# ga1i13o/DiffewS

Hardware: AMD Instinct MI355X
Metric: few-shot episodes/sec (512x512, 1-shot, SD-2 UNet) (higher is better)
Workload: dtype bf16; 1 GPU; SD-2.1 UNet + SD VAE, 512x512, 1-shot, 4 episodes/GPU/step (BASELINE.json configs[1]); nshot=1, resolution=512, parallelism=episode-sharded x1, hip_graph=True, residual_dtype=bf16, graph_owner=pipeline.run_episodes(captured=True)

## Files before the change

### diffews_amd/_lib.py

```python
import ctypes as C
import os

_HERE = os.path.dirname(os.path.abspath(__file__))
LIB_PATH = os.environ.get("DFW_LIB") or os.path.join(_HERE, "libdiffews_hip.so")

BF16, F16 = 0, 1
FILTER_BILINEAR, FILTER_BICUBIC = 0, 1
OUT_T, OUT_F32, OUT_NCHW_F32 = 0, 1, 2
ACT_NONE, ACT_SILU, ACT_CLAMP1 = 0, 1, 2

_vp, _i32, _i64, _f32, _sz = C.c_void_p, C.c_int32, C.c_int64, C.c_float, C.c_size_t


class GemmArgs(C.Structure):
    _fields_ = [("A", _vp), ("W", _vp), ("C", _vp), ("bias", _vp), ("rowbias", _vp), ("residual", _vp),
                ("workspace", _vp), ("workspace_bytes", _sz), ("a_elems", _i64), ("w_elems", _i64),
                ("M", _i32), ("N", _i32), ("K", _i32), ("lda", _i32), ("ldc", _i32), ("ldr", _i32), ("ld_rowbias", _i32),
                ("taps", _i32), ("Cin", _i32), ("Hi", _i32), ("Wi", _i32), ("Ho", _i32), ("Wo", _i32),
                ("stride", _i32), ("pad", _i32), ("ups", _i32), ("rows_per_img", _i32),
                ("out_scale", _f32), ("act", _i32), ("geglu", _i32), ("out_mode", _i32), ("splitk", _i32),
                ("batch", _i32), ("strideA", _i64), ("strideW", _i64), ("strideC", _i64), ("dtype", _i32),
                ("gn_partial", _vp), ("gn_groups", _i32),
                ("colscale", _f32), ("colscale_n", _i32), ("residual_f32", _i32), ("W_blocked", _vp)]

# ... 159 lines not shown
    _fields_ = [("q", _vp), ("k", _vp), ("v", _vp), ("out", _vp),
                ("batch", _i32), ("n", _i32), ("head_dim", _i32), ("q_prescaled", _i32),
                ("ldq", _i32), ("ldk", _i32), ("ldv", _i32), ("ldo", _i32),
                ("q_bs", _i64), ("k_bs", _i64), ("v_bs", _i64), ("o_bs", _i64), ("dtype", _i32)]


class AdamWArgs(C.Structure):
    _fields_ = [("param", _vp), ("grad", _vp), ("exp_avg", _vp), ("exp_avg_sq", _vp), ("grad_sumsq", _vp), ("n", _i64),
                ("lr", _f32), ("beta1", _f32), ("beta2", _f32), ("eps", _f32), ("weight_decay", _f32), ("max_grad_norm", _f32),
                ("step", _i32), ("shadow", _vp), ("shadow_dtype", _i32), ("found_inf", _vp)]


class Config(C.Structure):
    _fields_ = [("conv_patch", _i32), ("big_kernels", _i32), ("big_bm", _i32), ("big_bn", _i32), ("big_bk", _i32),
                ("gemm_bm", _i32), ("gemm_bn", _i32), ("fsa_key_split", _i32),
                ("fsa_force_splits", _i32), ("big_min_tiles", _i32), ("k8", _i32)]


SYMBOLS = {
    "dfw_configure": (_i32, [C.POINTER(Config)]),
    "dfw_get_config": (None, [C.POINTER(Config)]),
    "dfw_version": (_i32, []),
    "dfw_error_string": (C.c_char_p, [_i32]),
    "dfw_graph_memset_nodes": (_i32, [_vp, C.POINTER(_i32)]),
    "dfw_gemm": (_i32, [C.POINTER(GemmArgs), _vp]),
    "dfw_gemm_workspace_bytes": (_sz, [C.POINTER(GemmArgs)]),
    "dfw_gemm_kernel_name": (_i32, [C.POINTER(GemmArgs), C.c_char_p, _sz]),
    "dfw_gemm_gn_chunks": (_i32, [C.POINTER(GemmArgs)]),
    "dfw_conv_up2x": (_i32, [C.POINTER(ConvUp2xArgs), _vp]),
    "dfw_conv_up2x_kernel_name": (_i32, [C.POINTER(ConvUp2xArgs), C.c_char_p, _sz]),
    "dfw_conv_up2x_gn_chunks": (_i32, [C.POINTER(ConvUp2xArgs)]),
    "dfw_fsa_attention": (_i32, [C.POINTER(FsaArgs), _vp]),
    "dfw_fsa_workspace_bytes": (_sz, [C.POINTER(FsaArgs)]),
    "dfw_fsa_kernel_name": (_i32, [C.POINTER(FsaArgs), C.c_char_p, _sz]),
    "dfw_fsa_attention_sets": (_i32, [C.POINTER(FsaArgs), _i32, _vp]),
    "dfw_fsa_sets_kernel_name": (_i32, [C.POINTER(FsaArgs), _i32, C.c_char_p, _sz]),
    "dfw_fsa_attention_ragged": (_i32, [C.POINTER(FsaArgs), C.POINTER(_i32), _i32, _i32, _vp]),
    "dfw_fsa_ragged_kernel_name": (_i32, [C.POINTER(FsaArgs), C.POINTER(_i32), _i32, _i32, C.c_char_p, _sz]),
    "dfw_fsa_ragged_workspace_bytes": (_sz, [C.POINTER(FsaArgs), C.POINTER(_i32), _i32, _i32]),
    "dfw_fsa_attention_routed": (_i32, [C.POINTER(FsaArgs), _vp, C.POINTER(_i32), _i32, _i32, _vp]),
    "dfw_fsa_routed_kernel_name": (_i32, [C.POINTER(FsaArgs), _i32, _i32, C.c_char_p, _sz]),
    "dfw_fsa_routed_workspace_bytes": (_sz, [C.POINTER(FsaArgs), _i32, _i32]),
    "dfw_cross_attention": (_i32, [C.POINTER(XattnArgs), _vp]),
# ... 109 lines not shown
```

### diffews_amd/csrc/gemm.hip

```cpp
#include "gemm_common.h"
#include <stdio.h>
#include <stdlib.h>

namespace dfw {

template <typename T, int BM, int BN, bool CONV, bool RF32 = false>
__global__ __launch_bounds__(256, 2) void gemm_kernel(const GemmP p) {
  constexpr int WTM = BM / 2, WTN = BN / 2, MB = WTM / 32, NB = WTN / 32;
  constexpr int SA = BM / 32, SW = BN / 32;
  constexpr int BUF = (BM + BN) * 128;
  extern __shared__ __attribute__((aligned(16))) char smem[];

  const int tid = threadIdx.x, lane = tid & 63, wave = tid >> 6;
  const int wm = wave >> 1, wn = wave & 1;
  const int lr = lane & 31, lh = lane >> 5;

  const int ntiles = p.ntm * p.ntn;
  const int nxb = gridDim.x >> 3, xcd = blockIdx.x & 7;
  const int Q = (ntiles + 7) >> 3;
  const int t_end = min(ntiles, (xcd + 1) * Q);
  int tile = xcd * Q + (blockIdx.x >> 3);

  const int z = blockIdx.y;
  int ks0 = 0, ks1 = p.nk;
// ... 270 lines not shown
  const int zdim = p.batch > 1 ? p.batch : (p.splitk > 1 ? p.splitk : 1);
  int nwg = q.ntm * q.ntn;
  int cap = 256 * per_cu / (zdim < 4 ? zdim : 4);
  if (cap < 256) cap = 256;
  if (nwg > cap) nwg = cap;
  nwg = (nwg + 7) & ~7;
  dim3 grid(nwg, zdim);
  if (p.taps == 1) {
    if (pl.rf32) hipLaunchKernelGGL((gemm_kernel<T, BM, BN, false, true>), grid, dim3(256), lds, st, q);
    else hipLaunchKernelGGL((gemm_kernel<T, BM, BN, false>), grid, dim3(256), lds, st, q);
  } else {
    if (pl.rf32) hipLaunchKernelGGL((gemm_kernel<T, BM, BN, true, true>), grid, dim3(256), lds, st, q);
    else hipLaunchKernelGGL((gemm_kernel<T, BM, BN, true>), grid, dim3(256), lds, st, q);
  }
  DFW_CHECK_LAUNCH();
  if (p.splitk > 1) {
    const long long total = (long long)p.M * (p.N >> 2);
    int blocks = (int)((total + 255) / 256);
    if (blocks > 2048) blocks = 2048;
    hipLaunchKernelGGL((splitk_reduce_kernel<T>), dim3(blocks), dim3(256), 0, st, q);
    DFW_CHECK_LAUNCH();
  }
  return 0;
}

struct TileCost { int bm, bn; float R, L, E; };
static const TileCost kTiles[3] = {{128, 128, 1.67f, 0.70f, 0.f}, {128, 64, 2.8f, 0.50f, 0.f}, {64, 64, 3.7f, 0.40f, 0.f}};
static const TileCost kLinTiles[3] = {{128, 128, 5.29f, 0.312f, 1.94f}, {128, 64, 8.52f, 0.182f, 0.13f}, {64, 64, 12.9f, 0.145f, 0.f}};

static void plan_gemm(GemmP& p, int& bm, int& bn) {
  const int fbm = cfg().gemm_bm, fbn = cfg().gemm_bn;
  const bool fixed_sk = p.splitk >= 1;
  if (p.geglu) { bm = 128; bn = 128; p.splitk = 1; return; }
  const bool can_split = p.batch <= 1 && (p.N % 4) == 0;
  float best = 1e30f;
  int best_t = 0, best_sk = 1;
  for (int t = 0; t < 3; ++t) {
// ... 127 lines not shown
  p.splitk = splitk; p.batch = batch;
  p.res_f32 = a->residual_f32 ? 1 : 0;
  p.strideA = a->strideA; p.strideW = a->strideW; p.strideC = a->strideC;
  p.nk = a->K / 64; p.cpt = a->Cin / 64; p.ntn = 0; p.ntm = 0;
  p.dtype_bf16 = a->dtype == DFW_BF16;
  p.gn_partial = a->gn_partial; p.gn_groups = a->gn_groups; p.gn_chunks = 0;
#ifdef DFW_TILE_STAMPS
  p.stamps = nullptr; p.stamp_tiles = 0;
#endif
  p.conv_chunk_major = a->taps == 9 ? 1 : 0;
  if (p.splitk > p.nk) p.splitk = p.nk;
  plan_gemm(p, p.plan_bm, p.plan_bn);
  return 0;
}

static int plan_call(const dfw_gemm_args* a, GemmP& p, GemmPlan& pl) {
  const int rc = fill_params(a, p);
  if (rc == 0) pl = gemm_plan(p);
  return rc;
}

extern "C" int dfw_gemm_kernel_name(const dfw_gemm_args* a, char* buf, size_t n) {
  GemmP p;
  GemmPlan pl;
  const int rc = plan_call(a, p, pl);
  if (rc) return rc;
  if (!buf || n == 0) return DFW_EINVAL;
  const char *t = p.dtype_bf16 ? "bf16" : "f16", *k = p.taps == 9 ? "conv" : "lin";
  switch (pl.kernel) {
    case GemmKernel::K8: snprintf(buf, n, "gemm8_kernel<%s,256,%d,64,%s>", t, pl.bn, k); break;
// ... 37 lines not shown
```

### diffews_amd/csrc/gemm8.hip

```cpp
#include "gemm_common.h"
#include <type_traits>

namespace dfw {

template <typename T, bool CONV, int BN, bool UP2X = false>
__global__ __launch_bounds__(512, 2) void gemm8_kernel(const GemmP p) {
  constexpr int BM = 256, HT = 16384;
  static_assert(!UP2X || (CONV && BN != 160), "the folded upsample conv is a conv mode of the 256 / 128 wide tiles");
  constexpr int KW = UP2X ? 4 : 1;
  constexpr bool N160 = BN == 160;
  static_assert(!(N160 && CONV), "the 256 x 160 tile is instantiated for Linear shapes only");
  constexpr int WH = BN / 128;
  constexpr int WGN = N160 ? 2 : BN / 64, WGM = 8 / WGN;
  constexpr int NBW = N160 ? 5 : 4;
  constexpr int WTM = BM / WGM, MB6 = WTM / 16, MH = MB6 / 2;
  constexpr int WDMA = N160 ? 3 : 2 * WH;
  constexpr int WB160 = 65536, WS160 = 24576;
  constexpr int STG = N160 ? WB160 + 2 * WS160 : (2 + WH) * 32768;
  extern __shared__ __attribute__((aligned(16))) char smem[];
  const int tid = threadIdx.x, lane = tid & 63;
  const int wave = __builtin_amdgcn_readfirstlane(tid >> 6);
  const int wr = wave >> 2;
  const int wm = wave / WGN, wc = wave % WGN;
  const uint32_t lds0 = lds_addr(smem);

  const int ntiles = p.ntm * p.ntn;
  const int nxb = gridDim.x >> 3, xcd = blockIdx.x & 7;
  const int Q = (ntiles + 7) >> 3;
  const int t_end = min(ntiles, (xcd + 1) * Q);
  const int tile0 = xcd * Q + (blockIdx.x >> 3);
  if (tile0 >= t_end) return;
  const int my_tiles = (t_end - tile0 + nxb - 1) / nxb;
  const int nkt = p.K >> 6;
  const int cpt = p.Cin >> 6;

  const int z = blockIdx.y;
  const char* Ab = p.A;
  const char* Wb = p.W;
  char* Cb = p.C;
  if (p.batch > 1) {
    Ab += (size_t)z * p.strideA * sizeof(T);
    Wb += (size_t)z * p.strideW * sizeof(T);
    Cb += (size_t)z * p.strideC * sizeof(T);
  }
  const u32x4 ra = make_srd(Ab, p.a_bytes);
  const u32x4 rw = make_srd(Wb, p.w_bytes);

  auto tile_coords = [&](int t) -> TileC {
    TileC c;
    c.par = 0;
    if constexpr (UP2X) {
      c.par = t & 3;
      t >>= 2;
    }
    const int tn = t % p.ntn, tm = t / p.ntn;
    c.m0 = tm * BM;
    c.n0 = tn * BN;
    c.img = 0; c.oy0 = 0; c.ox0 = 0;
    if constexpr (CONV) {
      c.img = tm / p.tpi;
      const int t2 = tm - c.img * p.tpi, tyi = t2 / p.tpr, txi = t2 - tyi * p.tpr;
      c.oy0 = tyi << 4;
      c.ox0 = txi << 4;
    }
    return c;
  };
  auto row_to_m = [&](const TileC& c, int r) -> int {
    if constexpr (UP2X) return (c.img * p.Ho + 2 * (c.oy0 + (r >> 4)) + (c.par >> 1)) * p.Wo + 2 * (c.ox0 + (r & 15)) + (c.par & 1);
    else if constexpr (CONV) return (c.img * p.Ho + c.oy0 + (r >> 4)) * p.Wo + c.ox0 + (r & 15);
    else return c.m0 + r;
  };

  const int lrow = lane >> 3;
  const int kc = (lane & 7) ^ ((((wave & 1) << 2) + (lane >> 4)) & 7);
  const unsigned limH = p.ups ? 2 * p.Hi : p.Hi, limW = p.ups ? 2 * p.Wi : p.Wi;
  const int ush = p.ups ? 1 : 0;
  int a_kt = 0, a_ti = 0;
  bool a_live = true;
  uint32_t a_v0 = 0;
  int a_m = 0, a_ix0 = 0;
  int a_iy0 = 0;
  uint32_t a_pix = 0;
  auto a_setup = [&](const TileC& c) {
    if constexpr (!CONV) {
      a_m = c.m0 + wave * 8 + lrow;
      a_v0 = (uint32_t)(((size_t)a_m * p.lda + kc * 8) * sizeof(T));
    } else {
      a_iy0 = (c.oy0 + (wave >> 1)) * p.stride - p.pad;
      a_ix0 = (c.ox0 + (wave & 1) * 8 + lrow) * p.stride - p.pad;
      a_pix = (uint32_t)c.img * (uint32_t)(p.Hi * p.Wi);
      if constexpr (UP2X) {
        a_iy0 += c.par >> 1;
        a_ix0 += c.par & 1;
      }
    }
  };
  auto a_advance = [&]() {
    if (++a_kt == nkt) {
      a_kt = 0;
      if (++a_ti < my_tiles) a_setup(tile_coords(tile0 + a_ti * nxb));
      else a_live = false;
    }
  };
  auto issue_a = [&](int buf) __attribute__((always_inline)) {
    int ky = 0, kx = 0, cc = 0;
    if constexpr (UP2X) {
      cc = a_kt >> 2;
      ky = (a_kt >> 1) & 1;
      kx = a_kt & 1;
    } else if constexpr (CONV) {
      cc = a_kt / 9;
      const int tap = a_kt - cc * 9;
      ky = tap / 3;
      kx = tap - ky * 3;
    }
#pragma unroll
    for (int h = 0; h < 2; ++h) {
      const uint32_t dst = lds0 + (uint32_t)(h * 32768 + buf * HT) + (uint32_t)wave * 1024u;
#pragma unroll
      for (int j = 0; j < 2; ++j) {
        uint32_t off;
        if constexpr (!CONV) {
          const int dr = h * 128 + j * 64;
          off = (a_m + dr < p.M && a_live) ? a_v0 + (uint32_t)dr * (uint32_t)p.lda * (uint32_t)sizeof(T) + (uint32_t)a_kt * 128u : kOOB;
        } else {
          int iy = a_iy0 + (h * 8 + j * 4) * p.stride + ky, ix = a_ix0 + kx;
          const bool ok = (unsigned)iy < limH && (unsigned)ix < limW && a_live;
          iy >>= ush;
          ix >>= ush;
          off = ok ? ((a_pix + (uint32_t)(iy * p.Wi + ix)) * (uint32_t)p.lda + (uint32_t)(cc * 64 + kc * 8)) * (uint32_t)sizeof(T) : kOOB;
        }
        dma16(ra, off, dst + j * 8192);
      }
    }
    a_advance();
  };
  int w_kt = 0, w_ti = 0;
  bool w_live = true;
  uint32_t w_v0 = 0;
  int w_n = 0, w_par = 0;
  auto w_setup = [&](const TileC& c) {
    w_n = c.n0 + wave * 8 + lrow;
    w_par = c.par;
    w_v0 = (uint32_t)(((size_t)w_n * p.K * KW + kc * 8) * sizeof(T));
  };
  auto issue_w = [&](int buf) __attribute__((always_inline)) {
    uint32_t koff = (uint32_t)w_kt * 128u;
    if constexpr (UP2X) {
      const int cc = w_kt >> 2, tap = w_kt & 3;
      koff = (uint32_t)((w_par * 4 + tap) * p.Cin + cc * 64) * (uint32_t)sizeof(T);
    } else if constexpr (CONV) {
      const int cc = w_kt / 9, tap = w_kt - cc * 9;
      koff = (uint32_t)(tap * p.Cin + cc * 64) * (uint32_t)sizeof(T);
    }
    if constexpr (N160) {
      const uint32_t dst = lds0 + (uint32_t)(WB160 + buf * WS160) + (uint32_t)wave * 1024u;
#pragma unroll
      for (int j = 0; j < 3; ++j) {
// ... 1 lines not shown
        const bool ok = w_live && (j < 2 || wave < 4);
        dma16(rw, ok ? off : kOOB, dst + j * 8192);
      }
    }
#pragma unroll
    for (int h = 0; h < (N160 ? 0 : WH); ++h) {
      const uint32_t dst = lds0 + (uint32_t)((2 + h) * 32768 + buf * HT) + (uint32_t)wave * 1024u;
#pragma unroll
      for (int j = 0; j < 2; ++j) {
        const uint32_t off = w_v0 + (uint32_t)(h * 128 + j * 64) * (uint32_t)(p.K * KW) * (uint32_t)sizeof(T) + koff;
        bool ok = w_live;
        if constexpr (BN == 128) ok = ok && (w_n + j * 64 < p.N);
        dma16(rw, ok ? off : kOOB, dst + j * 8192);
      }
    }
    if (++w_kt == nkt) {
      w_kt = 0;
      if (++w_ti < my_tiles) {
        if (UP2X || p.ntn > 1) w_setup(tile_coords(tile0 + w_ti * nxb));
      } else w_live = false;
    }
  };

  uint32_t ab0, ab1, wb0, wb1;
  {
    const int l15 = lane & 15, l4 = lane >> 4;
    const uint32_t fb = (uint32_t)(l15 * 128 + ((l4 ^ (l15 >> 1)) << 4));
    ab0 = (uint32_t)(wr * 32768 + (wm % (WGM / 2)) * WTM * 128) + fb;
    ab1 = ab0 ^ 64u;
    if constexpr (N160) wb0 = (uint32_t)(WB160 + wc * 80 * 128) + fb;
    else wb0 = (uint32_t)((2 + (wc >> 1)) * 32768 + (wc & 1) * 64 * 128) + fb;
// ... 207 lines not shown
        s2 += __shfl_xor(s2, o, 64);
        q2 += __shfl_xor(q2, o, 64);
      }
      const int cp = lane & 31;
      if (lane < 32 && (cp & (ppg - 1)) == 0) {
        const int tm = (UP2X ? tile_id >> 2 : tile_id) / p.ntn;
        const int chunk = ((tm - c.img * p.tpi) * KW + c.par) * WGM + wm;
        const int grp = (c.n0 + wc * 64 + 2 * cp) / cpg;
        float* o2 = p.gn_partial + (((size_t)c.img * p.gn_chunks + chunk) * p.gn_groups + grp) * 2;
        o2[0] = s2;
        o2[1] = q2;
      }
    }
  };

  TileC ct = tile_coords(tile0);
  a_setup(ct);
  w_setup(ct);
  DFW_TILE_STAMP(p, wave, lane, 0, 0);
  issue_w(0);
  issue_a(0);
  issue_w(1);
  wait_vm<WDMA>();
  bar();
  if (wr == 1) bar();
  zero6();
  int kt = 0, ti = 0, buf = 0;
  const int total = my_tiles * nkt;
#pragma unroll 1
  for (int g = 0; g < total; ++g) {
    read_a(0);
    read_w(fw0, 0);
    read_w(fw1, 1);
    if constexpr (N160) read_w4();
    issue_a(buf ^ 1);
    lgkm0();
    bar();
    __builtin_amdgcn_s_setprio(1);
    mfmas(0, 0, fw0);
    mfmas(0, 1, fw1);
    if constexpr (N160) mfmas4(0);
    __builtin_amdgcn_s_setprio(0);
    bar();
    read_a(1);
    issue_w(buf);
    wait_vm<WDMA>();
    lgkm0();
    bar();
    __builtin_amdgcn_s_setprio(1);
    if constexpr (N160) mfmas4(1);
    mfmas(1, 1, fw1);
    mfmas(1, 0, fw0);
    __builtin_amdgcn_s_setprio(0);
    const bool last = kt + 1 == nkt;
    if (!(last && wr == 1)) bar();
    buf ^= 1;
    ab0 ^= (uint32_t)HT; ab1 ^= (uint32_t)HT;
    if constexpr (N160) { wb0 = wbase160 + (uint32_t)(buf * WS160); wb1 = wb0 ^ 64u; }
    else { wb0 ^= (uint32_t)HT; wb1 ^= (uint32_t)HT; }
    if (last) {
      DFW_TILE_STAMP(p, wave, lane, ti, 1);
      epilogue6(ct, smem + STG + wave * (N160 ? 5120 : 4096), tile0 + ti * nxb);
      DFW_TILE_STAMP(p, wave, lane, ti, 2);
      DFW_TILE_STAMP(p, wave, lane, ti + 1, 0);
      zero6();
      kt = 0;
      ++ti;
      if (ti < my_tiles) ct = tile_coords(tile0 + ti * nxb);
      if (wr == 1) bar();
    } else {
      ++kt;
    }
  }
  if (wr == 0) bar();
  wait_vm<0>();
}

template <typename T, int BN>
static int launch8(const GemmP& p, const GemmPlan& pl, hipStream_t st) {
  GemmP q = p;
  q.ntm = (p.M + 255) / 256;
  q.ntn = (p.N + BN - 1) / BN;
  q.gn_chunks = p.gn_partial ? pl.gn_chunks : 0;
// ... 73 lines not shown
  if (a->B <= 0 || a->Hi <= 0 || a->Wi <= 0 || a->Cin <= 0 || a->Cout <= 0 || a->x_elems <= 0 || a->w_elems <= 0) return DFW_EINVAL;
  if (a->dtype != DFW_BF16 && a->dtype != DFW_F16) return DFW_EINVAL;
  if (a->gn_groups < 0 || (a->gn_partial && a->gn_groups == 0)) return DFW_EINVAL;
  if ((a->Hi % 16) != 0 || (a->Wi % 16) != 0 || (a->Cin % 64) != 0 || (a->Cout % 64) != 0) return DFW_ESHAPE;
  if (a->ldx < a->Cin || (a->ldx % 8) != 0 || a->ldy < a->Cout || (a->ldy % 8) != 0) return DFW_ESHAPE;
  if (((uintptr_t)a->x & 15) || ((uintptr_t)a->W & 15) || ((uintptr_t)a->y & 15)) return DFW_ESHAPE;
  if ((a->bias && ((uintptr_t)a->bias & 15)) || (a->gn_partial && ((uintptr_t)a->gn_partial & 3))) return DFW_ESHAPE;
  const int64_t pix = (int64_t)a->B * a->Hi * a->Wi;
  if (a->x_elems * 2 >= (1ll << 31) || a->w_elems * 2 >= (1ll << 31) || 4 * pix >= (1ll << 31)) return DFW_ERANGE;
  if (a->x_elems < pix * a->ldx - (a->ldx - a->Cin) || a->w_elems < (int64_t)a->Cout * 16 * a->Cin) return DFW_EINVAL;
  bn = (a->Cout % 256) == 0 ? 256 : 128;
  if (a->gn_partial && up2x_gn_chunks(a, bn) == 0) return DFW_ESHAPE;
  return 0;
}

}

using namespace dfw;

extern "C" int dfw_conv_up2x_kernel_name(const dfw_conv_up2x_args* a, char* buf, size_t n) {
  if (!buf || n == 0) return DFW_EINVAL;
  buf[0] = 0;
  int bn = 0;
  const int rc = up2x_plan(a, bn);
  if (rc) return rc;
  snprintf(buf, n, "gemm8_kernel<%s,256,%d,64,up2x>", a->dtype == DFW_BF16 ? "bf16" : "f16", bn);
  return 0;
}

extern "C" int32_t dfw_conv_up2x_gn_chunks(const dfw_conv_up2x_args* a) {
  int bn = 0;
  if (!a) return 0;
  dfw_conv_up2x_args q = *a;
// ... 35 lines not shown
```

### diffews_amd/csrc/gemm_common.h

```cpp
#pragma once
#include "common.h"

namespace dfw {

struct GemmP {
  const char* A; const char* W; char* C;
  const char* Wblk;
  const float* bias; const float* rowbias; const char* residual; float* partial;
  uint32_t a_bytes, w_bytes;
  int M, N, K, lda, ldc, ldr, ldrb;
  int taps, Cin, Hi, Wi, Ho, Wo, stride, pad, ups, rows_per_img;
  float out_scale;
  float cs; int cs_n;
  int act, geglu, out_mode, splitk, batch;
  int res_f32;
  long long strideA, strideW, strideC;
  int nk, cpt, ntn, ntm;
  int plan_bm, plan_bn, dtype_bf16;
  float* gn_partial; int gn_groups, gn_chunks;
  int conv_chunk_major;
  int tw, tw_log2, tpr, tpi;
#ifdef DFW_TILE_STAMPS
  unsigned long long* stamps; int stamp_tiles;
#endif
// ... 248 lines not shown

struct TileC {
  int m0, n0;
  int img, oy0, ox0;
  int par;
};

enum class GemmKernel { Tile, Big, K8, Patch, Patch8 };
struct GemmPlan {
  GemmKernel kernel;
  int bm, bn, bk, splitk;
  int gn_chunks;
  bool f32o, rf32;
};

#define DFW_BY_DTYPE(p, ...) \
  ((p).dtype_bf16 ? [&] { using T = __bf16; return __VA_ARGS__; }() : [&] { using T = _Float16; return __VA_ARGS__; }())

}
```

### diffews_amd/csrc/misc.hip

```cpp
#include "common.h"
#include "seg_fuse.h"
#ifdef DFW_TILE_STAMPS
#include "gemm_common.h"
#endif
#include <stdio.h>
#include <stdlib.h>

namespace dfw {

struct CsP {
  const float* x; const float* W; const float* bias; char* y;
  int B, Cin, H, Wd, Cout, taps, ldy, out_mode;
  float in_scale, out_scale;
  int iters;
  float* gn_partial; int gn_groups, gn_chunks;
  long long ybs;
  const float* x1; const float* x2; int b0, b1;
};

__device__ __forceinline__ const float* cs_image(const CsP& p, int b) {
  const size_t per = (size_t)p.Cin * p.H * p.Wd;
  if (p.x1 == nullptr || b < p.b0) return p.x + (size_t)b * per;
  if (b < p.b1) return p.x1 + (size_t)(b - p.b0) * per;
  return p.x2 + (size_t)(b - p.b1) * per;
// ... 810 lines not shown
        cnt += c;
      }
    }
  }
  free(nodes);
  return cnt;
}

extern "C" int dfw_graph_memset_nodes(void* graph, int32_t* n_nodes) {
  if (!graph) return DFW_EINVAL;
  if (n_nodes) *n_nodes = 0;
  const int c = count_memset_nodes((hipGraph_t)graph, n_nodes, 0);
  return c < 0 ? DFW_EINVAL : c;
}

static const dfw_config kDefaultCfg = {3, 1, 0, 0, 0, 0, 0, 1, 0, 192, 3};
static dfw_config g_cfg = kDefaultCfg;
namespace dfw { const dfw_config& cfg() { return g_cfg; } }

extern "C" int dfw_configure(const dfw_config* c) {
  if (!c) { g_cfg = kDefaultCfg; return 0; }
  if (c->conv_patch < 0 || c->conv_patch > 4 || c->fsa_force_splits < 0 || c->big_min_tiles < 1 || c->k8 < 0 || c->k8 > 3) return DFW_EINVAL;
  if (c->gemm_bm && !((c->gemm_bm == 128 && (c->gemm_bn == 128 || c->gemm_bn == 64)) || (c->gemm_bm == 64 && c->gemm_bn == 64))) return DFW_EINVAL;
  g_cfg = *c;
  return 0;
}

extern "C" void dfw_get_config(dfw_config* out) {
  if (out) *out = g_cfg;
}

#ifdef DFW_TILE_STAMPS
static dfw::TileStampCfg g_stamps = {nullptr, 0, 0};
namespace dfw { const TileStampCfg& tile_stamp_cfg() { return g_stamps; } }
extern "C" int dfw_debug_tile_stamps(void* buf, int32_t tiles, int32_t grid_cap) {
  if (tiles < 0 || grid_cap < 0 || (grid_cap & 7) || (buf && tiles == 0)) return DFW_EINVAL;
  g_stamps = {(unsigned long long*)buf, buf ? tiles : 0, grid_cap};
  return 0;
}
#endif

extern "C" int dfw_version(void) { return 114; }

extern "C" const char* dfw_error_string(int code) {
  switch (code) {
    case 0: return "success";
    case DFW_EINVAL: return "invalid argument (null pointer or non-positive size)";
    case DFW_ESHAPE: return "shape not supported by the gfx950 kernel (alignment / multiple-of constraint)";
    case DFW_ERANGE: return "tensor exceeds the 2 GiB buffer-descriptor range";
    case DFW_EWORKSPACE: return "workspace missing or too small";
    default: return code > 0 ? hipGetErrorString((hipError_t)code) : "unknown error";
  }
}
```

### diffews_amd/ops.py

```python
import ctypes as C
import os
import math

import torch

from . import _lib as L

_DT = {torch.bfloat16: L.BF16, torch.float16: L.F16}


def _stream():
    return C.c_void_p(torch.cuda.current_stream().cuda_stream)


def _p(t):
    return C.c_void_p(t.data_ptr()) if t is not None else None


def _dt(t):
    try:
        return _DT[t.dtype]
    except KeyError:
        raise TypeError(f"engine storage dtype must be bfloat16 or float16, got {t.dtype}")

# ... 3 lines not shown
        raise TypeError(f"{name} must be a contiguous float32 tensor")
    return t


def _rowbias(a, rb):
    if rb is None:
        return
    if rb.dtype != torch.float32 or rb.dim() != 2 or rb.stride(1) != 1:
        raise TypeError("rowbias must be float32 [imgs, N] with unit column stride")
    a.rowbias, a.ld_rowbias = rb.data_ptr(), rb.stride(0)


gemm_hook = None


def _gemm_call(a):
    lib = L.lib()
    if gemm_hook is not None:
        buf = C.create_string_buffer(64)
        L.check(lib.dfw_gemm_kernel_name(C.byref(a), buf, 64), "dfw_gemm_kernel_name")
        _timed(buf.value.decode(), 2.0 * a.M * a.N * a.K * max(1, a.batch),
               (a.M, a.N, a.K, a.taps, a.stride, a.ups, a.splitk, max(1, a.batch)), lambda: _gemm_launch(lib, a))
        return
    _gemm_launch(lib, a)


def _gemm_launch(lib, a):
    nbytes = lib.dfw_gemm_workspace_bytes(C.byref(a))
    if nbytes:
        ws = torch.empty(nbytes // 4, dtype=torch.float32, device="cuda")
        a.workspace, a.workspace_bytes = ws.data_ptr(), nbytes
    L.check(lib.dfw_gemm(C.byref(a), _stream()), "dfw_gemm")
    return


def linear(x, w, bias=None, residual=None, rowbias=None, rows_per_img=0, act=L.ACT_NONE, geglu=False,
           out=None, out_f32=False, out_scale=1.0, splitk=None, colscale=None):
    assert x.dim() == 2 and w.dim() == 2 and x.stride(1) == 1 and w.is_contiguous()
    M, K = x.shape
    N = w.shape[0]
    assert w.shape[1] == K and w.dtype == x.dtype
    n_out = N // 2 if geglu else N
    if out is None:
        out = torch.empty(M, n_out, dtype=torch.float32 if out_f32 else x.dtype, device=x.device)
    assert out.stride(1) == 1 and out.shape == (M, n_out)
    a = L.GemmArgs()
    a.A, a.W, a.C = x.data_ptr(), w.data_ptr(), out.data_ptr()
# ... 27 lines not shown
    a.A, a.W, a.C = x.data_ptr(), w.data_ptr(), out.data_ptr()
    a.a_elems, a.w_elems = M * K, N * K
    a.M, a.N, a.K, a.lda, a.ldc = M, N, K, K, N
    a.taps, a.Cin = 1, K
    a.out_scale = out_scale
    a.out_mode = L.OUT_F32 if out_f32 else L.OUT_T
    a.splitk, a.batch = 1, Bt
    a.strideA, a.strideW, a.strideC = M * K, N * K, M * N
    a.dtype = _dt(x)
    _gemm_call(a)
    return out


def conv3x3(x, w, cout, bias=None, stride=1, pad=1, ups=False, rowbias=None, residual=None,
            out_nchw_f32=False, out_scale=1.0, splitk=None, gn_groups=0, gn_in=None, act=L.ACT_NONE,
            out_f32=False, w_blk=None):
    assert x.dim() == 4 and x.stride(3) == 1 and x.is_contiguous()
    B, Hi, Wi, Cin = x.shape
    if gn_in is not None:
        x = groupnorm(x, *gn_in, out_dtype=w.dtype)
    assert w.shape == (cout, 9 * Cin) and w.dtype == x.dtype and w.is_contiguous()
    if ups:
        assert stride == 1 and pad == 1
        Ho, Wo = 2 * Hi, 2 * Wi
    elif stride == 1:
        Ho, Wo = Hi, Wi
    else:
        Ho, Wo = (Hi + 2 * pad - 3) // stride + 1 if pad else Hi // 2, (Wi + 2 * pad - 3) // stride + 1 if pad else Wi // 2
    M = B * Ho * Wo
    if out_nchw_f32:
        out = torch.empty(B, cout, Ho, Wo, dtype=torch.float32, device=x.device)
# ... 8 lines not shown
    _rowbias(a, rowbias)
    if residual is not None:
        assert residual.dtype in (x.dtype, torch.float32) and residual.is_contiguous() and residual.numel() == M * cout
        a.residual, a.ldr = residual.data_ptr(), cout
        a.residual_f32 = int(residual.dtype == torch.float32)
    a.a_elems, a.w_elems = x.numel(), w.numel()
    a.M, a.N, a.K, a.lda, a.ldc = M, cout, 9 * Cin, Cin, cout
    a.taps, a.Cin, a.Hi, a.Wi, a.Ho, a.Wo = 9, Cin, Hi, Wi, Ho, Wo
    a.stride, a.pad, a.ups = stride, pad, int(ups)
    a.rows_per_img = Ho * Wo
    a.out_scale, a.act = out_scale, act
    a.out_mode = L.OUT_NCHW_F32 if out_nchw_f32 else (L.OUT_F32 if out_f32 else L.OUT_T)
    a.splitk = 0 if splitk is None else splitk
    a.batch, a.dtype = 1, _dt(x)
    stats = None
    if gn_groups and not out_nchw_f32:
        a.gn_groups = gn_groups
        chunks = L.lib().dfw_gemm_gn_chunks(C.byref(a))
        if chunks > 0:
            part = torch.empty(B, chunks, gn_groups, 2, dtype=torch.float32, device=x.device)
            a.gn_partial = part.data_ptr()
            stats = (part, chunks, gn_groups)
    _gemm_call(a)
    if stats is not None:
        out._gn_stats = stats
    return out


def _timed(name, flops, shape, call):
    e0, e1 = torch.cuda.Event(enable_timing=True), torch.cuda.Event(enable_timing=True)
    e0.record()
    call()
    e1.record()
    gemm_hook(name, flops, e0, e1, shape)


def _fsa_args(q, k, v, out, heads):
    B, N, Cq = q.shape
# ... 137 lines not shown
    lo = torch.empty(x.shape, dtype=dtype, device=x.device)
    L.check(L.lib().dfw_split_f32(x.data_ptr(), hi.data_ptr(), lo.data_ptr(), x.numel(), _DT[dtype], _stream()), "dfw_split_f32")
    return hi, lo


def linear_stream(x, w, bias=None, residual=None):
    if x.dtype != torch.float32:
        return linear(x, w, bias=bias, residual=residual)
    hi, lo = split_storage(x, w.dtype)
    y = linear(hi, w, bias=bias, residual=residual, out_f32=True)
    return linear(lo, w, residual=y, out_f32=True)


def conv3x3_stream(x, w, cout, bias=None, lo=True, w_up2x=None, **kw):
    if x.dtype != torch.float32:
        if w_up2x is not None and UP2X_FOLD and kw.get("ups") and set(kw) <= {"ups", "gn_groups"}:
            y = conv3x3_up2x(x, w_up2x, cout, bias=bias, gn_groups=kw.get("gn_groups", 0))
            if y is not None:
                return y
        return conv3x3(x, w, cout, bias=bias, **kw)
    if not lo:
        return conv3x3(to_storage(x, w.dtype), w, cout, bias=bias, out_f32=True, **kw)
    hi, lo = split_storage(x, w.dtype)
    gn_groups = kw.pop("gn_groups", 0)
    y = conv3x3(hi, w, cout, bias=bias, out_f32=True, **kw)
    return conv3x3(lo, w, cout, residual=y, out_f32=True, gn_groups=gn_groups, **kw)


UP2X_FOLD = True


# ... 536 lines not shown
```

### diffews_amd/unet.py

```python
from dataclasses import dataclass

import os

import torch

from . import _lib as L
from . import ops, ops_bwd, packing, weights


@dataclass
class UNet2DConditionOutput:
    sample: torch.Tensor = None


class _Cfg(dict):
    __getattr__ = dict.__getitem__


def _resolve_device(d):
    d = torch.device(d)
    if d.type == "cuda" and d.index is None:
        d = torch.device("cuda", torch.cuda.current_device() if torch.cuda.is_available() else 0)
    return d

# ... 26 lines not shown
        self.ws = None
        if p + "conv_shortcut.weight" in sd:
            self.ws = packing.pack_conv1x1(g("conv_shortcut.weight")).to(dev, dt)
            self.bs = g("conv_shortcut.bias").float().to(dev)
        self.has_temb = p + "time_emb_proj.weight" in sd
        self.temb_slice = None

    def __call__(self, x, tproj=None):
        B, H, W, Cin = x.shape
        dt, f32s = self.w1.dtype, x.dtype == torch.float32
        h = ops.groupnorm(x, self.g1, self.b1, self.groups, self.eps, silu=True, out_dtype=dt)
        rb = None
        if self.has_temb:
            o, c = self.temb_slice
            rb = tproj[:, o:o + c]
        h = ops.conv3x3(h, self.w1, self.cout, bias=self.cb1, rowbias=rb, gn_groups=self.groups)
        h = ops.groupnorm(h, self.g2, self.b2, self.groups, self.eps, silu=True)
        sc = x
        if self.ws is not None:
            sc = ops.linear_stream(x.view(-1, Cin), self.ws, bias=self.bs).view(B, H, W, self.cout)
        return ops.conv3x3(h, self.w2, self.cout, bias=self.cb2, residual=sc, gn_groups=self.groups, out_f32=f32s)


def bank_layout(config, h, w):
    boc = list(config["block_out_channels"])
    lpb = config["layers_per_block"]
    sizes = [(h, w)]
    for _ in boc[1:]:
        sizes.append(((sizes[-1][0] + 1) // 2, (sizes[-1][1] + 1) // 2))
    out = []
    for i, typ in enumerate(config["down_block_types"]):
        if typ == "CrossAttnDownBlock2D":
            out += [(sizes[i][0] * sizes[i][1], boc[i])] * lpb
    for i, typ in enumerate(config["up_block_types"]):
        if typ == "CrossAttnUpBlock2D":
            j = len(boc) - 1 - i
# ... 680 lines not shown
            if blk["down"] is not None:
                d = blk["down"]
                x = ops.conv3x3_stream(x, d.w, d.cout, bias=d.b, stride=2, pad=1)
                skips.append(x)
        x = self.mid["res"][0](x, tproj)
        x = self.mid["attn"](x, ehs2d, L_ctx, n_ref, bank_io)
        x = self.mid["res"][1](x, tproj)
        for blk in self.up:
            for j, r in enumerate(blk["res"]):
                x = ops.concat_channels(x, skips.pop())
                x = r(x, tproj)
                if blk["attn"] is not None:
                    x = blk["attn"][j](x, ehs2d, L_ctx, n_ref, bank_io)
            if blk["up"] is not None:
                u = blk["up"]
                x = ops.conv3x3_stream(x, u.w, u.cout, bias=u.b, ups=True)
        x = ops.groupnorm(x, *self.gn_out, self.groups, self.eps, silu=True, out_dtype=self.dtype)
        co = self.conv_out
        return ops.conv3x3(x, co.w, co.cout, bias=co.b, out_nchw_f32=True, out_scale=out_scale)


CustomUNet2DConditionModel = MyUNet2DConditionModel
```

### include/diffews_hip.h

```cpp
#ifndef DIFFEWS_HIP_H
#define DIFFEWS_HIP_H

#include <stddef.h>
#include <stdint.h>

#ifdef __cplusplus
extern "C" {
#endif

typedef void* dfw_stream_t;

enum { DFW_BF16 = 0, DFW_F16 = 1 };
enum { DFW_OUT_T = 0, DFW_OUT_F32 = 1, DFW_OUT_NCHW_F32 = 2 };
enum { DFW_ACT_NONE = 0, DFW_ACT_SILU = 1, DFW_ACT_CLAMP1 = 2  };
enum {
  DFW_EINVAL = -1,
  DFW_ESHAPE = -2,
  DFW_ERANGE = -3,
  DFW_EWORKSPACE = -4
};

int dfw_version(void);
const char* dfw_error_string(int code);

typedef struct {
  int32_t conv_patch;
  int32_t big_kernels;
  int32_t big_bm, big_bn, big_bk;
  int32_t gemm_bm, gemm_bn;
  int32_t fsa_key_split;
  int32_t fsa_force_splits;
  int32_t big_min_tiles;
  int32_t k8;
} dfw_config;
int dfw_configure(const dfw_config* cfg);
void dfw_get_config(dfw_config* out);

int dfw_graph_memset_nodes(void* hip_graph, int32_t* n_nodes);

typedef struct {
  const void* A; const void* W; void* C;
  const float* bias; const float* rowbias; const void* residual;
  void* workspace; size_t workspace_bytes;
  int64_t a_elems, w_elems;
  int32_t M, N, K;
  int32_t lda, ldc, ldr;
  int32_t ld_rowbias;
  int32_t taps, Cin, Hi, Wi, Ho, Wo, stride, pad, ups;
  int32_t rows_per_img;
  float out_scale;
  int32_t act, geglu, out_mode, splitk;
  int32_t batch; int64_t strideA, strideW, strideC;
  int32_t dtype;
  float* gn_partial; int32_t gn_groups;
  float colscale; int32_t colscale_n;
  int32_t residual_f32;
  const void* W_blocked;
} dfw_gemm_args;

int dfw_gemm(const dfw_gemm_args* a, dfw_stream_t stream);
size_t dfw_gemm_workspace_bytes(const dfw_gemm_args* a);
int dfw_gemm_kernel_name(const dfw_gemm_args* a, char* buf, size_t n);
int32_t dfw_gemm_gn_chunks(const dfw_gemm_args* a);

typedef struct {
  const void* x; const void* W; void* y; const float* bias;
  int64_t x_elems, w_elems;
  int32_t B, Hi, Wi, Cin, Cout;
  int32_t ldx, ldy;
  int32_t dtype;
  float* gn_partial; int32_t gn_groups;
} dfw_conv_up2x_args;

int dfw_conv_up2x(const dfw_conv_up2x_args* a, dfw_stream_t stream);
int dfw_conv_up2x_kernel_name(const dfw_conv_up2x_args* a, char* buf, size_t n);
int32_t dfw_conv_up2x_gn_chunks(const dfw_conv_up2x_args* a);

typedef struct {
// ... 436 lines not shown
```

Before: 104.5 episodes/s.

## Add K-slab split-K mode to 256-row conv kernel for small spatial maps

Adds a split-K variant of the 256x128 conv3x3 gemm8 kernel for 8x8 and 16x16 feature maps. It slices the K dimension into slabs, writes fp32 partials to a workspace and reduces them with the existing split-K reduce kernel. This targets the low-resolution UNet resnet and upsample convs, which have few output tiles and leave most CUs idle. The cost is extra fp32 partial traffic, an additional reduce launch, and the loss of fused GroupNorm partial stats on those convs.

Result: no change. 105.1 episodes/s, median of 6 (+0.6%).

```diff
diff --git a/diffews_amd/_lib.py b/diffews_amd/_lib.py
--- a/diffews_amd/_lib.py
+++ b/diffews_amd/_lib.py
@@ -197,7 +197,7 @@
 class Config(C.Structure):
     _fields_ = [("conv_patch", _i32), ("big_kernels", _i32), ("big_bm", _i32), ("big_bn", _i32), ("big_bk", _i32),
                 ("gemm_bm", _i32), ("gemm_bn", _i32), ("fsa_key_split", _i32),
-                ("fsa_force_splits", _i32), ("big_min_tiles", _i32), ("k8", _i32)]
+                ("fsa_force_splits", _i32), ("big_min_tiles", _i32), ("k8", _i32), ("kslab", _i32)]
 
 
 SYMBOLS = {
@@ -210,6 +210,9 @@
     "dfw_gemm_workspace_bytes": (_sz, [C.POINTER(GemmArgs)]),
     "dfw_gemm_kernel_name": (_i32, [C.POINTER(GemmArgs), C.c_char_p, _sz]),
     "dfw_gemm_gn_chunks": (_i32, [C.POINTER(GemmArgs)]),
+    "dfw_conv_kslab": (_i32, [C.POINTER(GemmArgs), _vp]),
+    "dfw_conv_kslab_workspace_bytes": (_sz, [C.POINTER(GemmArgs)]),
+    "dfw_conv_kslab_kernel_name": (_i32, [C.POINTER(GemmArgs), C.c_char_p, _sz]),
     "dfw_conv_up2x": (_i32, [C.POINTER(ConvUp2xArgs), _vp]),
     "dfw_conv_up2x_kernel_name": (_i32, [C.POINTER(ConvUp2xArgs), C.c_char_p, _sz]),
     "dfw_conv_up2x_gn_chunks": (_i32, [C.POINTER(ConvUp2xArgs)]),
diff --git a/diffews_amd/csrc/gemm.hip b/diffews_amd/csrc/gemm.hip
--- a/diffews_amd/csrc/gemm.hip
+++ b/diffews_amd/csrc/gemm.hip
@@ -308,13 +308,17 @@
     else hipLaunchKernelGGL((gemm_kernel<T, BM, BN, true>), grid, dim3(256), lds, st, q);
   }
   DFW_CHECK_LAUNCH();
-  if (p.splitk > 1) {
-    const long long total = (long long)p.M * (p.N >> 2);
-    int blocks = (int)((total + 255) / 256);
-    if (blocks > 2048) blocks = 2048;
-    hipLaunchKernelGGL((splitk_reduce_kernel<T>), dim3(blocks), dim3(256), 0, st, q);
-    DFW_CHECK_LAUNCH();
-  }
+  if (p.splitk > 1) return launch_splitk_reduce(q, st);
+  return 0;
+}
+
+int launch_splitk_reduce(const GemmP& p, hipStream_t st) {
+  const long long total = (long long)p.M * (p.N >> 2);
+  int blocks = (int)((total + 255) / 256);
+  if (blocks > 2048) blocks = 2048;
+  if (p.dtype_bf16) hipLaunchKernelGGL((splitk_reduce_kernel<__bf16>), dim3(blocks), dim3(256), 0, st, p);
+  else hipLaunchKernelGGL((splitk_reduce_kernel<_Float16>), dim3(blocks), dim3(256), 0, st, p);
+  DFW_CHECK_LAUNCH();
   return 0;
 }
 
@@ -472,6 +476,8 @@
   return 0;
 }
 
+namespace dfw { int gemm_fill_params(const dfw_gemm_args* a, GemmP& p) { return fill_params(a, p); } }
+
 static int plan_call(const dfw_gemm_args* a, GemmP& p, GemmPlan& pl) {
   const int rc = fill_params(a, p);
   if (rc == 0) pl = gemm_plan(p);
diff --git a/diffews_amd/csrc/gemm8.hip b/diffews_amd/csrc/gemm8.hip
--- a/diffews_amd/csrc/gemm8.hip
+++ b/diffews_amd/csrc/gemm8.hip
@@ -3,10 +3,11 @@
 
 namespace dfw {
 
-template <typename T, bool CONV, int BN, bool UP2X = false>
+template <typename T, bool CONV, int BN, bool UP2X = false, bool KSLAB = false>
 __global__ __launch_bounds__(512, 2) void gemm8_kernel(const GemmP p) {
   constexpr int BM = 256, HT = 16384;
   static_assert(!UP2X || (CONV && BN != 160), "the folded upsample conv is a conv mode of the 256 / 128 wide tiles");
+  static_assert(!KSLAB || (CONV && !UP2X && BN != 160), "K slabs are a conv mode of the 256 / 128 wide tiles");
   constexpr int KW = UP2X ? 4 : 1;
   constexpr bool N160 = BN == 160;
   static_assert(!(N160 && CONV), "the 256 x 160 tile is instantiated for Linear shapes only");
@@ -24,7 +25,8 @@
   const int wm = wave / WGN, wc = wave % WGN;
   const uint32_t lds0 = lds_addr(smem);
 
-  const int ntiles = p.ntm * p.ntn;
+  int ntiles = p.ntm * p.ntn;
+  if constexpr (KSLAB) ntiles *= p.splitk;
   const int nxb = gridDim.x >> 3, xcd = blockIdx.x & 7;
   const int Q = (ntiles + 7) >> 3;
   const int t_end = min(ntiles, (xcd + 1) * Q);
@@ -33,6 +35,10 @@
   const int my_tiles = (t_end - tile0 + nxb - 1) / nxb;
   const int nkt = p.K >> 6;
   const int cpt = p.Cin >> 6;
+  const int sl_base = KSLAB ? nkt / p.splitk : 0, sl_rem = KSLAB ? nkt - sl_base * p.splitk : 0;
+  const bool map8 = KSLAB && p.tw == 8;
+  auto slice_k0 = [&](int s) -> int { return s * sl_base + min(s, sl_rem); };
+  auto slice_len = [&](int s) -> int { return sl_base + (s < sl_rem ? 1 : 0); };
 
   const int z = blockIdx.y;
   const char* Ab = p.A;
@@ -53,21 +59,31 @@
       c.par = t & 3;
       t >>= 2;
     }
-    const int tn = t % p.ntn, tm = t / p.ntn;
+    int tn = t % p.ntn, tm = t / p.ntn;
+    if constexpr (KSLAB) {
+      tm = t % p.ntm;
+      t /= p.ntm;
+      c.par = t % p.splitk;
+      tn = t / p.splitk;
+    }
     c.m0 = tm * BM;
     c.n0 = tn * BN;
     c.img = 0; c.oy0 = 0; c.ox0 = 0;
     if constexpr (CONV) {
-      c.img = tm / p.tpi;
-      const int t2 = tm - c.img * p.tpi, tyi = t2 / p.tpr, txi = t2 - tyi * p.tpr;
-      c.oy0 = tyi << 4;
-      c.ox0 = txi << 4;
+      if (map8) {
+        c.img = tm << 2;
+      } else {
+        c.img = tm / p.tpi;
+        const int t2 = tm - c.img * p.tpi, tyi = t2 / p.tpr, txi = t2 - tyi * p.tpr;
+        c.oy0 = tyi << 4;
+        c.ox0 = txi << 4;
+      }
     }
     return c;
   };
   auto row_to_m = [&](const TileC& c, int r) -> int {
     if constexpr (UP2X) return (c.img * p.Ho + 2 * (c.oy0 + (r >> 4)) + (c.par >> 1)) * p.Wo + 2 * (c.ox0 + (r & 15)) + (c.par & 1);
-    else if constexpr (CONV) return (c.img * p.Ho + c.oy0 + (r >> 4)) * p.Wo + c.ox0 + (r & 15);
+    else if constexpr (CONV) return map8 ? c.m0 + r : (c.img * p.Ho + c.oy0 + (r >> 4)) * p.Wo + c.ox0 + (r & 15);
     else return c.m0 + r;
   };
 
@@ -81,6 +97,7 @@
   int a_m = 0, a_ix0 = 0;
   int a_iy0 = 0;
   uint32_t a_pix = 0;
+  int a_end = 0, a_nimg = 4;
   auto a_setup = [&](const TileC& c) {
     if constexpr (!CONV) {
       a_m = c.m0 + wave * 8 + lrow;
@@ -89,6 +106,15 @@
       a_iy0 = (c.oy0 + (wave >> 1)) * p.stride - p.pad;
       a_ix0 = (c.ox0 + (wave & 1) * 8 + lrow) * p.stride - p.pad;
       a_pix = (uint32_t)c.img * (uint32_t)(p.Hi * p.Wi);
+      if constexpr (KSLAB) {
+        a_kt = slice_k0(c.par);
+        a_end = a_kt + slice_len(c.par);
+        if (map8) {
+          a_iy0 = wave * p.stride - p.pad;
+          a_ix0 = lrow * p.stride - p.pad;
+          a_nimg = (p.M >> 6) - c.img;
+        }
+      }
       if constexpr (UP2X) {
         a_iy0 += c.par >> 1;
         a_ix0 += c.par & 1;
@@ -96,7 +122,12 @@
     }
   };
   auto a_advance = [&]() {
-    if (++a_kt == nkt) {
+    if constexpr (KSLAB) {
+      if (++a_kt == a_end) {
+        if (++a_ti < my_tiles) a_setup(tile_coords(tile0 + a_ti * nxb));
+        else a_live = false;
+      }
+    } else if (++a_kt == nkt) {
       a_kt = 0;
       if (++a_ti < my_tiles) a_setup(tile_coords(tile0 + a_ti * nxb));
       else a_live = false;
@@ -125,10 +156,18 @@
           off = (a_m + dr < p.M && a_live) ? a_v0 + (uint32_t)dr * (uint32_t)p.lda * (uint32_t)sizeof(T) + (uint32_t)a_kt * 128u : kOOB;
         } else {
           int iy = a_iy0 + (h * 8 + j * 4) * p.stride + ky, ix = a_ix0 + kx;
-          const bool ok = (unsigned)iy < limH && (unsigned)ix < limW && a_live;
+          bool ok = (unsigned)iy < limH && (unsigned)ix < limW && a_live;
+          uint32_t pix = a_pix;
+          if constexpr (KSLAB) {
+            if (map8) {
+              iy = a_iy0 + ky;
+              ok = (unsigned)iy < limH && (unsigned)ix < limW && a_live && (h * 2 + j) < a_nimg;
+              pix += (uint32_t)((h * 2 + j) * p.Hi * p.Wi);
+            }
+          }
           iy >>= ush;
           ix >>= ush;
-          off = ok ? ((a_pix + (uint32_t)(iy * p.Wi + ix)) * (uint32_t)p.lda + (uint32_t)(cc * 64 + kc * 8)) * (uint32_t)sizeof(T) : kOOB;
+          off = ok ? ((pix + (uint32_t)(iy * p.Wi + ix)) * (uint32_t)p.lda + (uint32_t)(cc * 64 + kc * 8)) * (uint32_t)sizeof(T) : kOOB;
         }
         dma16(ra, off, dst + j * 8192);
       }
@@ -138,10 +177,14 @@
   int w_kt = 0, w_ti = 0;
   bool w_live = true;
   uint32_t w_v0 = 0;
-  int w_n = 0, w_par = 0;
+  int w_n = 0, w_par = 0, w_end = 0;
   auto w_setup = [&](const TileC& c) {
     w_n = c.n0 + wave * 8 + lrow;
     w_par = c.par;
+    if constexpr (KSLAB) {
+      w_kt = slice_k0(c.par);
+      w_end = w_kt + slice_len(c.par);
+    }
     w_v0 = (uint32_t)(((size_t)w_n * p.K * KW + kc * 8) * sizeof(T));
   };
   auto issue_w = [&](int buf) __attribute__((always_inline)) {
@@ -173,7 +216,12 @@
         dma16(rw, ok ? off : kOOB, dst + j * 8192);
       }
     }
-    if (++w_kt == nkt) {
+    if constexpr (KSLAB) {
+      if (++w_kt == w_end) {
+        if (++w_ti < my_tiles) w_setup(tile_coords(tile0 + w_ti * nxb));
+        else w_live = false;
+      }
+    } else if (++w_kt == nkt) {
       w_kt = 0;
       if (++w_ti < my_tiles) {
         if (UP2X || p.ntn > 1) w_setup(tile_coords(tile0 + w_ti * nxb));
@@ -411,6 +459,19 @@
     }
   };
 
+  auto slab_store = [&](const TileC& c) {
+    if (c.n0 + wc * 64 >= p.N) return;
+    const int l15 = lane & 15, l4 = lane >> 4;
+    float* const sl = p.partial + (size_t)c.par * (size_t)p.M * (size_t)p.N + (c.n0 + wc * 64 + 4 * l4);
+#pragma unroll
+    for (int b = 0; b < MB6; ++b) {
+      const int m = row_to_m(c, wm * WTM + b * 16 + l15);
+      if (m >= p.M) continue;
+#pragma unroll
+      for (int j = 0; j < NBW; ++j) *(f32x4*)(sl + (size_t)m * (size_t)p.N + j * 16) = acc6[b][j];
+    }
+  };
+
   TileC ct = tile_coords(tile0);
   a_setup(ct);
   w_setup(ct);
@@ -423,7 +484,12 @@
   if (wr == 1) bar();
   zero6();
   int kt = 0, ti = 0, buf = 0;
-  const int total = my_tiles * nkt;
+  int total = my_tiles * nkt, ukt = nkt;
+  if constexpr (KSLAB) {
+    total = 0;
+    for (int i = 0; i < my_tiles; ++i) total += slice_len(tile_coords(tile0 + i * nxb).par);
+    ukt = slice_len(ct.par);
+  }
 #pragma unroll 1
   for (int g = 0; g < total; ++g) {
     read_a(0);
@@ -449,7 +515,7 @@
     mfmas(1, 1, fw1);
     mfmas(1, 0, fw0);
     __builtin_amdgcn_s_setprio(0);
-    const bool last = kt + 1 == nkt;
+    const bool last = kt + 1 == ukt;
     if (!(last && wr == 1)) bar();
     buf ^= 1;
     ab0 ^= (uint32_t)HT; ab1 ^= (uint32_t)HT;
@@ -457,13 +523,17 @@
     else { wb0 ^= (uint32_t)HT; wb1 ^= (uint32_t)HT; }
     if (last) {
       DFW_TILE_STAMP(p, wave, lane, ti, 1);
-      epilogue6(ct, smem + STG + wave * (N160 ? 5120 : 4096), tile0 + ti * nxb);
+      if constexpr (KSLAB) slab_store(ct);
+      else epilogue6(ct, smem + STG + wave * (N160 ? 5120 : 4096), tile0 + ti * nxb);
       DFW_TILE_STAMP(p, wave, lane, ti, 2);
       DFW_TILE_STAMP(p, wave, lane, ti + 1, 0);
       zero6();
       kt = 0;
       ++ti;
-      if (ti < my_tiles) ct = tile_coords(tile0 + ti * nxb);
+      if (ti < my_tiles) {
+        ct = tile_coords(tile0 + ti * nxb);
+        if constexpr (KSLAB) ukt = slice_len(ct.par);
+      }
       if (wr == 1) bar();
     } else {
       ++kt;
@@ -567,9 +637,86 @@
   return 0;
 }
 
+constexpr int kSlabKMin = 8;
+constexpr int kSlabBN = 128;
+
+static int kslab_plan(const dfw_gemm_args* a, GemmP& p) {
+  const int rc = gemm_fill_params(a, p);
+  if (rc) return rc;
+  if (!cfg().kslab || !cfg().k8) return DFW_ESHAPE;
+  if (p.taps != 9 || p.stride != 1 || p.pad != 1 || p.batch > 1 || p.geglu) return DFW_ESHAPE;
+  if (p.out_mode != DFW_OUT_T || p.res_f32 || p.gn_partial) return DFW_ESHAPE;
+  if ((p.Cin % 64) != 0 || (p.N % 64) != 0) return DFW_ESHAPE;
+  const bool up = p.ups != 0;
+  if (p.Ho != (up ? 2 * p.Hi : p.Hi) || p.Wo != (up ? 2 * p.Wi : p.Wi)) return DFW_ESHAPE;
+  const bool map8 = p.Ho == 8 && p.Wo == 8;
+  if (!map8 && (p.Ho != 16 || p.Wo != 16)) return DFW_ESHAPE;
+  if (((uintptr_t)p.A & 15) || ((uintptr_t)p.W & 15) || ((uintptr_t)p.C & 15) || (p.ldc % 4) != 0) return DFW_ESHAPE;
+  if (p.M < 256) return DFW_ESHAPE;
+  p.ntm = (p.M + 255) / 256;
+  p.ntn = (p.N + kSlabBN - 1) / kSlabBN;
+  const int units = p.ntm * p.ntn, nkt = p.K / 64;
+  int S;
+  if (a->splitk >= 2) {
+    S = a->splitk;
+    if (S > 64 || nkt / S < 2) return DFW_ESHAPE;
+  } else {
+    S = 256 / units;
+    if (S > nkt / kSlabKMin) S = nkt / kSlabKMin;
+    if (S < 2) return DFW_ESHAPE;
+  }
+  p.splitk = S;
+  p.tw = map8 ? 8 : 16; p.tw_log2 = map8 ? 3 : 4;
+  p.tpr = map8 ? 1 : p.Wo / 16;
+  p.tpi = map8 ? 1 : p.tpr * (p.Ho / 16);
+  p.gn_partial = nullptr; p.gn_chunks = 0;
+  return 0;
+}
+
+template <typename T>
+static int launch_kslab(const GemmP& p0, hipStream_t st) {
+  constexpr size_t lds = (size_t)(2 + kSlabBN / 128) * 32768 + 32768;
+  GemmP p = p0;
+  int nwg = p.ntm * p.ntn * p.splitk;
+  if (nwg > 256) nwg = 256;
+  nwg = (nwg + 7) & ~7;
+  DFW_STAMP_LAUNCH(p, nwg);
+  auto kfn = gemm8_kernel<T, true, kSlabBN, false, true>;
+  (void)hipFuncSetAttribute((const void*)kfn, hipFuncAttributeMaxDynamicSharedMemorySize, (int)lds);
+  hipLaunchKernelGGL(kfn, dim3(nwg), dim3(512), lds, st, p);
+  DFW_CHECK_LAUNCH();
+  return launch_splitk_reduce(p, st);
+}
+
 }
 
 using namespace dfw;
+
+extern "C" size_t dfw_conv_kslab_workspace_bytes(const dfw_gemm_args* a) {
+  GemmP p;
+  if (kslab_plan(a, p)) return 0;
+  return (size_t)p.splitk * (size_t)p.M * (size_t)p.N * sizeof(float);
+}
+
+extern "C" int dfw_conv_kslab_kernel_name(const dfw_gemm_args* a, char* buf, size_t n) {
+  if (!buf || n == 0) return DFW_EINVAL;
+  buf[0] = 0;
+  GemmP p;
+  const int rc = kslab_plan(a, p);
+  if (rc) return rc;
+  snprintf(buf, n, "gemm8_kernel<%s,256,%d,64,conv>+kslab", p.dtype_bf16 ? "bf16" : "f16", kSlabBN);
+  return 0;
+}
+
+extern "C" int dfw_conv_kslab(const dfw_gemm_args* a, dfw_stream_t stream) {
+  GemmP p;
+  const int rc = kslab_plan(a, p);
+  if (rc) return rc;
+  const size_t need = (size_t)p.splitk * (size_t)p.M * (size_t)p.N * sizeof(float);
+  if (!a->workspace || a->workspace_bytes < need || ((uintptr_t)a->workspace & 15)) return DFW_EWORKSPACE;
+  hipStream_t st = (hipStream_t)stream;
+  return DFW_BY_DTYPE(p, launch_kslab<T>(p, st));
+}
 
 extern "C" int dfw_conv_up2x_kernel_name(const dfw_conv_up2x_args* a, char* buf, size_t n) {
   if (!buf || n == 0) return DFW_EINVAL;
diff --git a/diffews_amd/csrc/gemm_common.h b/diffews_amd/csrc/gemm_common.h
--- a/diffews_amd/csrc/gemm_common.h
+++ b/diffews_amd/csrc/gemm_common.h
@@ -286,6 +286,9 @@
   bool f32o, rf32;
 };
 
+int gemm_fill_params(const dfw_gemm_args* a, GemmP& p);
+int launch_splitk_reduce(const GemmP& p, hipStream_t st);
+
 #define DFW_BY_DTYPE(p, ...) \
   ((p).dtype_bf16 ? [&] { using T = __bf16; return __VA_ARGS__; }() : [&] { using T = _Float16; return __VA_ARGS__; }())
 
diff --git a/diffews_amd/csrc/misc.hip b/diffews_amd/csrc/misc.hip
--- a/diffews_amd/csrc/misc.hip
+++ b/diffews_amd/csrc/misc.hip
@@ -848,13 +848,13 @@
   return c < 0 ? DFW_EINVAL : c;
 }
 
-static const dfw_config kDefaultCfg = {3, 1, 0, 0, 0, 0, 0, 1, 0, 192, 3};
+static const dfw_config kDefaultCfg = {3, 1, 0, 0, 0, 0, 0, 1, 0, 192, 3, 1};
 static dfw_config g_cfg = kDefaultCfg;
 namespace dfw { const dfw_config& cfg() { return g_cfg; } }
 
 extern "C" int dfw_configure(const dfw_config* c) {
   if (!c) { g_cfg = kDefaultCfg; return 0; }
-  if (c->conv_patch < 0 || c->conv_patch > 4 || c->fsa_force_splits < 0 || c->big_min_tiles < 1 || c->k8 < 0 || c->k8 > 3) return DFW_EINVAL;
+  if (c->conv_patch < 0 || c->conv_patch > 4 || c->fsa_force_splits < 0 || c->big_min_tiles < 1 || c->k8 < 0 || c->k8 > 3 || c->kslab < 0 || c->kslab > 1) return DFW_EINVAL;
   if (c->gemm_bm && !((c->gemm_bm == 128 && (c->gemm_bn == 128 || c->gemm_bn == 64)) || (c->gemm_bm == 64 && c->gemm_bn == 64))) return DFW_EINVAL;
   g_cfg = *c;
   return 0;
@@ -874,7 +874,7 @@
 }
 #endif
 
-extern "C" int dfw_version(void) { return 114; }
+extern "C" int dfw_version(void) { return 115; }
 
 extern "C" const char* dfw_error_string(int code) {
   switch (code) {
diff --git a/diffews_amd/ops.py b/diffews_amd/ops.py
--- a/diffews_amd/ops.py
+++ b/diffews_amd/ops.py
@@ -41,23 +41,28 @@
 gemm_hook = None
 
 
-def _gemm_call(a):
+def _gemm_call(a, kslab=False):
     lib = L.lib()
     if gemm_hook is not None:
         buf = C.create_string_buffer(64)
-        L.check(lib.dfw_gemm_kernel_name(C.byref(a), buf, 64), "dfw_gemm_kernel_name")
+        if kslab:
+            L.check(lib.dfw_conv_kslab_kernel_name(C.byref(a), buf, 64), "dfw_conv_kslab_kernel_name")
+        else:
+            L.check(lib.dfw_gemm_kernel_name(C.byref(a), buf, 64), "dfw_gemm_kernel_name")
         _timed(buf.value.decode(), 2.0 * a.M * a.N * a.K * max(1, a.batch),
-               (a.M, a.N, a.K, a.taps, a.stride, a.ups, a.splitk, max(1, a.batch)), lambda: _gemm_launch(lib, a))
+               (a.M, a.N, a.K, a.taps, a.stride, a.ups, a.splitk, max(1, a.batch)), lambda: _gemm_launch(lib, a, kslab))
         return
-    _gemm_launch(lib, a)
-
-
-def _gemm_launch(lib, a):
-    nbytes = lib.dfw_gemm_workspace_bytes(C.byref(a))
+    _gemm_launch(lib, a, kslab)
+
+
+def _gemm_launch(lib, a, kslab=False):
+    query, launch, what = ((lib.dfw_conv_kslab_workspace_bytes, lib.dfw_conv_kslab, "dfw_conv_kslab") if kslab else
+                           (lib.dfw_gemm_workspace_bytes, lib.dfw_gemm, "dfw_gemm"))
+    nbytes = query(C.byref(a))
     if nbytes:
         ws = torch.empty(nbytes // 4, dtype=torch.float32, device="cuda")
         a.workspace, a.workspace_bytes = ws.data_ptr(), nbytes
-    L.check(lib.dfw_gemm(C.byref(a), _stream()), "dfw_gemm")
+    L.check(launch(C.byref(a), _stream()), what)
     return
 
 
@@ -115,7 +120,7 @@
 
 def conv3x3(x, w, cout, bias=None, stride=1, pad=1, ups=False, rowbias=None, residual=None,
             out_nchw_f32=False, out_scale=1.0, splitk=None, gn_groups=0, gn_in=None, act=L.ACT_NONE,
-            out_f32=False, w_blk=None):
+            out_f32=False, w_blk=None, kslab=False):
     assert x.dim() == 4 and x.stride(3) == 1 and x.is_contiguous()
     B, Hi, Wi, Cin = x.shape
     if gn_in is not None:
@@ -154,14 +159,18 @@
     a.splitk = 0 if splitk is None else splitk
     a.batch, a.dtype = 1, _dt(x)
     stats = None
-    if gn_groups and not out_nchw_f32:
+    kslab = bool(kslab) and L.lib().dfw_conv_kslab_workspace_bytes(C.byref(a)) > 0
+    if gn_groups and not out_nchw_f32 and not kslab:
         a.gn_groups = gn_groups
         chunks = L.lib().dfw_gemm_gn_chunks(C.byref(a))
         if chunks > 0:
             part = torch.empty(B, chunks, gn_groups, 2, dtype=torch.float32, device=x.device)
             a.gn_partial = part.data_ptr()
             stats = (part, chunks, gn_groups)
-    _gemm_call(a)
+    if kslab:
+        _gemm_call(a, True)
+    else:
+        _gemm_call(a)
     if stats is not None:
         out._gn_stats = stats
     return out
@@ -329,7 +338,7 @@
 
 def conv3x3_stream(x, w, cout, bias=None, lo=True, w_up2x=None, **kw):
     if x.dtype != torch.float32:
-        if w_up2x is not None and UP2X_FOLD and kw.get("ups") and set(kw) <= {"ups", "gn_groups"}:
+        if w_up2x is not None and UP2X_FOLD and kw.get("ups") and set(kw) <= {"ups", "gn_groups", "kslab"}:
             y = conv3x3_up2x(x, w_up2x, cout, bias=bias, gn_groups=kw.get("gn_groups", 0))
             if y is not None:
                 return y
diff --git a/diffews_amd/unet.py b/diffews_amd/unet.py
--- a/diffews_amd/unet.py
+++ b/diffews_amd/unet.py
@@ -64,12 +64,12 @@
         if self.has_temb:
             o, c = self.temb_slice
             rb = tproj[:, o:o + c]
-        h = ops.conv3x3(h, self.w1, self.cout, bias=self.cb1, rowbias=rb, gn_groups=self.groups)
+        h = ops.conv3x3(h, self.w1, self.cout, bias=self.cb1, rowbias=rb, gn_groups=self.groups, kslab=not f32s)
         h = ops.groupnorm(h, self.g2, self.b2, self.groups, self.eps, silu=True)
         sc = x
         if self.ws is not None:
             sc = ops.linear_stream(x.view(-1, Cin), self.ws, bias=self.bs).view(B, H, W, self.cout)
-        return ops.conv3x3(h, self.w2, self.cout, bias=self.cb2, residual=sc, gn_groups=self.groups, out_f32=f32s)
+        return ops.conv3x3(h, self.w2, self.cout, bias=self.cb2, residual=sc, gn_groups=self.groups, out_f32=f32s, kslab=True)
 
 
 def bank_layout(config, h, w):
@@ -780,7 +780,7 @@
                     x = blk["attn"][j](x, ehs2d, L_ctx, n_ref, bank_io)
             if blk["up"] is not None:
                 u = blk["up"]
-                x = ops.conv3x3_stream(x, u.w, u.cout, bias=u.b, ups=True)
+                x = ops.conv3x3_stream(x, u.w, u.cout, bias=u.b, ups=True, kslab=True)
         x = ops.groupnorm(x, *self.gn_out, self.groups, self.eps, silu=True, out_dtype=self.dtype)
         co = self.conv_out
         return ops.conv3x3(x, co.w, co.cout, bias=co.b, out_nchw_f32=True, out_scale=out_scale)
diff --git a/include/diffews_hip.h b/include/diffews_hip.h
--- a/include/diffews_hip.h
+++ b/include/diffews_hip.h
@@ -32,6 +32,7 @@
   int32_t fsa_force_splits;
   int32_t big_min_tiles;
   int32_t k8;
+  int32_t kslab;
 } dfw_config;
 int dfw_configure(const dfw_config* cfg);
 void dfw_get_config(dfw_config* out);
@@ -62,6 +63,10 @@
 size_t dfw_gemm_workspace_bytes(const dfw_gemm_args* a);
 int dfw_gemm_kernel_name(const dfw_gemm_args* a, char* buf, size_t n);
 int32_t dfw_gemm_gn_chunks(const dfw_gemm_args* a);
+
+int dfw_conv_kslab(const dfw_gemm_args* a, dfw_stream_t stream);
+size_t dfw_conv_kslab_workspace_bytes(const dfw_gemm_args* a);
+int dfw_conv_kslab_kernel_name(const dfw_gemm_args* a, char* buf, size_t n);
 
 typedef struct {
   const void* x; const void* W; void* y; const float* bias;
```
